# awikner/SPEEDY-ML-1

Measured on AMD Instinct MI355X. Metric: hybrid timesteps/sec, T30L8 + 1152x6k-node reservoirs; 1/2/4/8-GPU scaling, higher is better.
Workload: dtype f64

## Files before the change

### speedy-ml-1_amd/csrc/sml_dynamics.hip

```cpp
#include <hip/hip_runtime.h>

#include <array>
#include <cmath>
#include <cstddef>
#include <cstdlib>
#include <cstring>
#include <new>
#include <utility>
#include <vector>

#include "sml_dynamics_tables.hpp"
#include "sml_fft.hpp"
#include "sml_fft_wa96.hpp"
#include "sml_physics.hpp"
#include "sml_physics_pair.hpp"
#include "sml_spectral_internal.hpp"
#include "sml_timeline.hpp"

SML_TL_DEFINE(dynamics)

using namespace sml;

namespace {

// ... 385 lines not shown
    SML_TAB_NM(X)
#undef X
    __device__ double gradx_m() const { return t->gradx; }
    __device__ double xc(int k1, int k) const { return t->xc[k1][k]; }
    __device__ double xd(int k1, int k) const { return t->xd[k1][k]; }
    __device__ double xj(int n, int k1, int k) const { return t->xj[k1][k][n]; }
};

__host__ __device__ inline double tabm_value(const DynTables *__restrict__ T, int m, int i) {
    const TabM *z = nullptr;
    const size_t off = (size_t)i * sizeof(double);
#define X(name)                                                                             \
    {                                                                                       \
        const size_t a = offsetof(TabM, name), b = a + sizeof(z->name);                      \
        if (off >= a && off < b) return T->name[(off - a) / sizeof(double)];                 \
    }
    SML_TAB_VEC(X)
#undef X
#define X(name)                                                                             \
    {                                                                                       \
        const size_t a = offsetof(TabM, name), b = a + sizeof(z->name);                      \
        if (off >= a && off < b) return T->name[(off - a) / sizeof(double)][m];              \
    }
    SML_TAB_NM(X)
#undef X
    if (off >= offsetof(TabM, xc) && off < offsetof(TabM, xc) + sizeof(z->xc))
        return (&T->xc[0][0])[(off - offsetof(TabM, xc)) / sizeof(double)];
    if (off >= offsetof(TabM, xd) && off < offsetof(TabM, xd) + sizeof(z->xd))
        return (&T->xd[0][0])[(off - offsetof(TabM, xd)) / sizeof(double)];
    if (off == offsetof(TabM, gradx)) return T->gradx[m];
    if (off >= offsetof(TabM, xj)) {
        const int q = (int)((off - offsetof(TabM, xj)) / sizeof(double));
        const int k1 = q / (kKX * kNX), k = (q / kNX) % kKX, n = q % kNX;
        return m + n >= 1 ? T->xj[m + n - 1][k1][k] : 0.0;
    }
    return 0.0;
}

template <class U, class V, class TB>
__device__ inline void vds_gen(U u, V v, const TB &tb, int n, int p, double *vor, double *div) {
    const double gx = tb.gradx_m();
    const double ux = u(1 - p, n), vx = v(1 - p, n);
    const double zp = p == 1 ? gx * ux : -gx * ux;
    const double zc = p == 1 ? gx * vx : -gx * vx;
    static_assert(kNTRUN1 - 1 == kNX - 2, "vds's last row reads n - 1");
    const int nm = n > 0 ? n - 1 : 0, np = n < kNX - 1 ? n + 1 : kNX - 1;
    const double um = u(p, nm), up = u(p, np), vm = v(p, nm), vp = v(p, np);
    const double dym = tb.vddym_n(n), dyp = tb.vddyp_n(n);
    const double vor0 = zc - dyp * up, div0 = zp + dyp * vp;
    const double vorl = dym * um, divl = -dym * vm;
    const double vori = dym * um - dyp * up + zc, divi = -dym * vm + dyp * vp + zp;
    *vor = n == 0 ? vor0 : n == kNX - 1 ? vorl : vori;
    *div = n == 0 ? div0 : n == kNX - 1 ? divl : divi;
}

__device__ inline void vds_at(const double *u, const double *v, const DynTables *T, int m, int n, int p, double *vor,
                              double *div) {
    vds_gen([&](int pp, int nn) { return u[ci(pp, m, nn)]; }, [&](int pp, int nn) { return v[ci(pp, m, nn)]; },
            GTab{T, m}, n, p, vor, div);
}

__global__ void k_dyn_combine(const double *__restrict__ S, double *__restrict__ Td, const DynTables *__restrict__ T) {
    const int mn = blockIdx.x * blockDim.x + threadIdx.x;
    if (mn >= kMN) return;
    const int k = blockIdx.y;
    const int m = mn % kMX, n = mn / kMX;
    auto fld = [&](int f) { return S + (size_t)f * kSF; };
#pragma unroll
    for (int p = 0; p < 2; ++p) {
        const int c = ci(p, m, n);
        double vo, dv, d0, dq, dummy;
        vds_at(fld(k), fld(3 * kKX + k), T, m, n, p, &vo, &dv);
        const double lapv = -(fld(6 * kKX + k)[c] * T->el2[n][m]);
        Td[kTVor + (size_t)k * kSF + c] = vo;
        Td[kTDiv + (size_t)k * kSF + c] = dv - lapv;
        vds_at(fld(kKX + k), fld(4 * kKX + k), T, m, n, p, &dummy, &d0);
        Td[kTT + (size_t)k * kSF + c] = d0 + fld(7 * kKX + k)[c];
        vds_at(fld(2 * kKX + k), fld(5 * kKX + k), T, m, n, p, &dummy, &dq);
        Td[kTTr + (size_t)k * kSF + c] = dq + fld(8 * kKX + k)[c];
        if (k == 0) Td[kTPs + c] = (m == 0 && n == 0) ? 0.0 : fld(kNFwd - 1)[c];
    }
}

template <int CW, bool KU, class SA, class TB>
__device__ inline void tail_coef(SA S, double *__restrict__ Td, double *__restrict__ phi_out,
                                 const double *__restrict__ phis, const double *__restrict__ tcorh,
                                 const double *__restrict__ qcorh, int fc, const TB &tb,
                                 double (*sh)[kKX][CW], int cc, int k, int c, int m, int n, double vordt, double divdt,
                                 double tdt, double trdt, double psdt, int j1, int j4, double dt, double alph,
                                 double rob, double wil) {
    sh[0][k][cc] = S(1, j4, k);
    sh[1][k][cc] = S(2, j4, k);
    __syncthreads();
    double d0[kKX], dh[kKX], t1[kKX], g1[kKX], g2[kKX];
#pragma unroll
    for (int kk = 0; kk < kKX; ++kk) {
        d0[kk] = sh[0][kk][cc];
        dh[kk] = tb.dhs(kk);
        t1[kk] = sh[1][kk][cc];
        g1[kk] = tb.xgeop1(kk);
        g2[kk] = kk > 0 ? tb.xgeop2(kk) : 0.0;
    }
    const int km = k > 0 ? k - 1 : 0, kp = k < kKX - 1 ? k + 1 : kKX - 1;
    const double trk = tb.tref(k), trm = tb.tref(km), trp = tb.tref(kp), dhsr_k = tb.dhsr(k), tref3_k = tb.tref3(k),
                 tref2_k = tb.tref2(k), phis_c = phis[fc], corf_k = tb.corf(k);
    double dmeanc = 0.0;
#pragma unroll
    for (int kk = 0; kk < kKX; ++kk) dmeanc = dmeanc + d0[kk] * dh[kk];
    psdt = psdt - dmeanc;
    if (m == 0 && n == 0) psdt = 0.0;
    double sig_k = 0.0, sig_k1 = 0.0;
    if constexpr (KU) {
        double sg = 0.0, sgp = 0.0;
#pragma unroll
        for (int kk = 0; kk < kKX - 1; ++kk) {
            if (kk > k) break;
            const double nx_ = sg - dh[kk] * (d0[kk] - dmeanc);
            sgp = sg;
            sg = nx_;
        }
        if (k == kKX - 1) {
            sig_k = sg;
        } else {
            sig_k = sgp;
            sig_k1 = sg;
        }
    } else {
        double sg = 0.0;
#pragma unroll
        for (int kk = 0; kk < kKX - 1; ++kk) {
            const double nx_ = sg - dh[kk] * (d0[kk] - dmeanc);
            if (kk == k - 1) sig_k = nx_;
            if (kk == k) sig_k1 = nx_;
            sg = nx_;
        }
    }
    const double dumk_k = (k == 0) ? 0.0 : sig_k * (trk - trm);
    const double dumk_k1 = (k == kKX - 1) ? 0.0 : sig_k1 * (trp - trk);
    tdt = tdt - (dumk_k1 + dumk_k) * dhsr_k + tref3_k * (sig_k1 + sig_k) - tref2_k * dmeanc;
    double phi = phis_c + g1[kKX - 1] * t1[kKX - 1];
#pragma unroll
    for (int kk = kKX - 2; kk >= 0; --kk) {
        if constexpr (KU)
            if (kk < k) break;
        const double nx = phi + g2[kk + 1] * t1[kk + 1] + g1[kk] * t1[kk];
        phi = kk >= k ? nx : phi;
    }
    {
        const double pc = phi + corf_k * (sh[1][kp][cc] - sh[1][km][cc]);
        if (m == 0 && k >= 1 && k <= kKX - 2) phi = pc;
    }
    if (phi_out) phi_out[(size_t)k * kSF + c] = phi;
    {
        const double d1 = phi + kRgas * trk * S(4, j4, 0);
        const double lapd = -(d1 * tb.el2_n(n));
        divdt = divdt - lapd;
    }
    if (alph != 0.0) {
        sh[2][k][cc] = tdt;
        __syncthreads();
        double ye = 0.0;
#pragma unroll
        for (int k1 = 0; k1 < kKX; ++k1) ye = ye + tb.xd(k1, k) * sh[2][k1][cc];
        ye = ye + tb.tref1(k) * psdt;
        sh[1][k][cc] = divdt + tb.elz_n(n) * ye;
        __syncthreads();
        divdt = 0.0;
        const int ll = m + n;
        if (ll != 0) {
#pragma unroll
            for (int k1 = 0; k1 < kKX; ++k1) divdt = divdt + tb.xj(n, k1, k) * sh[1][k1][cc];
        }
        sh[0][k][cc] = divdt;
        __syncthreads();
#pragma unroll
        for (int kk = 0; kk < kKX; ++kk) psdt = psdt - sh[0][kk][cc] * tb.dhsx(kk);
#pragma unroll
        for (int k1 = 0; k1 < kKX; ++k1) tdt = tdt + tb.xc(k1, k) * sh[0][k1][cc];
    }
    const double dmp = tb.dmp_n(n), dmp1 = tb.dmp1_n(n), dmpd = tb.dmpd_n(n), dmp1d = tb.dmp1d_n(n);
    vordt = (vordt - dmp * S(0, 1, k)) * dmp1;
    divdt = (divdt - dmpd * S(1, 1, k)) * dmp1d;
    const double ctmp = S(2, 1, k) + tcorh[fc] * tb.tcorv(k);
    tdt = (tdt - dmp * ctmp) * dmp1;
    if (k == 0) {
        if (m == 0) {
            const double sdrag = 1. / (kTdrs * 3600.);
            vordt = vordt - sdrag * S(0, 1, 0);
            divdt = divdt - sdrag * S(1, 1, 0);
        }
        const double dmps = tb.dmps_n(n), dmp1s = tb.dmp1s_n(n);
        vordt = (vordt - dmps * S(0, 1, 0)) * dmp1s;
        divdt = (divdt - dmps * S(1, 1, 0)) * dmp1s;
        tdt = (tdt - dmps * ctmp) * dmp1s;
    }
    {
        const double cq = S(3, 1, k) + qcorh[fc] * tb.qcorv(k);
        trdt = (trdt - dmpd * cq) * dmp1d;
    }
    if (dt <= 0.0) {
        if (!Td) return;
        Td[kTVor + (size_t)k * kSF + c] = vordt;
        Td[kTDiv + (size_t)k * kSF + c] = divdt;
        Td[kTT + (size_t)k * kSF + c] = tdt;
        Td[kTTr + (size_t)k * kSF + c] = trdt;
        if (k == 0) Td[kTPs + c] = psdt;
        return;
    }
    const double eps = (j1 == 1) ? 0.0 : rob;
    const double trf = tb.trfilt_n(n);
    auto timint = [&](int var, int kk, double fdt) {
        fdt = fdt * trf;
        double &f1 = S(var, 1, kk);
        double &f2 = S(var, 2, kk);
        const double fj1_old = (j1 == 1) ? f1 : f2;
        const double fnew = f1 + dt * fdt;
        const double f1new = fj1_old + wil * eps * (f1 - 2 * fj1_old + fnew);
        const double fj1_new = (j1 == 1) ? f1new : fj1_old;
        f2 = fnew - (1 - wil) * eps * (f1new - 2 * fj1_new + fnew);
        f1 = f1new;
    };
    if (k == 0) timint(4, 0, psdt);
    timint(0, k, vordt);
    timint(1, k, divdt);
    timint(2, k, tdt);
    timint(3, k, trdt);
}

constexpr int kTailC = 32;
__global__ __launch_bounds__(256) void k_dyn_tail(double *__restrict__ st, double *__restrict__ Td,
                                                  double *__restrict__ phi_out, const double *__restrict__ phis,
                                                  const double *__restrict__ tcorh, const double *__restrict__ qcorh,
                                                  const DynTables *__restrict__ T, int j1, int j4, double dt,
                                                  double alph, double rob, double wil) {
    __shared__ double sh[3][kKX][kTailC];
    const int cc = threadIdx.x & (kTailC - 1), k = threadIdx.x / kTailC;
    const int c = blockIdx.x * kTailC + cc;
    const int mn = c >> 1, m = mn % kMX, n = mn / kMX;
    auto S = [&](int var, int lev, int kk) -> double & {
        if (var == 4) return st[kOffPs + (size_t)(lev - 1) * kSF + c];
        const size_t off = var == 0 ? kOffVor : var == 1 ? kOffDiv : var == 2 ? kOffT : kOffTr;
        return st[off + ((size_t)(lev - 1) * kKX + kk) * kSF + c];
    };
    tail_coef<kTailC, false>(S, Td, phi_out, phis, tcorh, qcorh, c, GTab{T, m}, sh, cc, k, c, m, n,
                             Td[kTVor + (size_t)k * kSF + c], Td[kTDiv + (size_t)k * kSF + c],
                             Td[kTT + (size_t)k * kSF + c], Td[kTTr + (size_t)k * kSF + c], Td[kTPs + c], j1, j4, dt,
                             alph, rob, wil);
}

typedef double d4 __attribute__((ext_vector_type(4)));
#define MFMA64(a, b, c) __builtin_amdgcn_mfma_f64_16x16x4f64((a), (b), (c), 0, 0, 0)

__device__ __attribute__((always_inline)) inline void store2(double *base, size_t idx, double a, double b) {
    *reinterpret_cast<double2 *>(base + idx) = double2{a, b};
}

constexpr int kCW = 2 * kNX;
static_assert(kCW == 64, "one level per 64-lane wave: wave_index() is the level index of the per-m kernels");
__device__ inline int wave_index() { return __builtin_amdgcn_readfirstlane((int)(threadIdx.x >> 6)); }
constexpr int kNIo = 4 * kKX + 1;
constexpr int kNIoWind = 2 * kKX;
constexpr int kSM = 5 * 2 * kKX * kCW;
constexpr int kVLs = 2 * kNFwd;
constexpr int kVFm = kIL * kVLs;
constexpr int kVIl = 2 * kNInvMax;
constexpr int kVIm = kIL * kVIl;
__device__ inline int smi(int var, int lev, int k, int cc) { return ((var * 2 + lev - 1) * kKX + k) * kCW + cc; }

constexpr int kStampKernels = 4, kStampBlocks = 96, kStamps = 8;
__device__ inline void stamp(long long *dbg, int kern, int i) {
    if (dbg && threadIdx.x == 0) dbg[((size_t)kern * kStampBlocks + blockIdx.x) * kStamps + i] = wall_clock64();
}

__global__ void k_state_to_m(const double *__restrict__ st, double *__restrict__ sm) {
    const int e = blockIdx.x * blockDim.x + threadIdx.x;
    if (e >= kMX * kSM) return;
    const int m = e / kSM, i = e % kSM;
    const int cc = i % kCW, k = (i / kCW) % kKX, lev = (i / (kCW * kKX)) % 2, var = i / (2 * kKX * kCW);
    const int c = ci(cc & 1, m, cc >> 1);
    double v = 0.0;
    if (var < 4) {
        const size_t off = var == 0 ? kOffVor : var == 1 ? kOffDiv : var == 2 ? kOffT : kOffTr;
        v = st[off + ((size_t)lev * kKX + k) * kSF + c];
    } else if (k == 0) {
        v = st[kOffPs + (size_t)lev * kSF + c];
    }
    sm[e] = v;
}

__device__ inline void put_state(double *__restrict__ st, int m, int i, double v) {
    const int cc = i % kCW, k = (i / kCW) % kKX, lev = (i / (kCW * kKX)) % 2, var = i / (2 * kKX * kCW);
    const int c = ci(cc & 1, m, cc >> 1);
    if (var < 4) {
        const size_t off = var == 0 ? kOffVor : var == 1 ? kOffDiv : var == 2 ? kOffT : kOffTr;
        st[off + ((size_t)lev * kKX + k) * kSF + c] = v;
    } else if (k == 0) {
        st[kOffPs + (size_t)lev * kSF + c] = v;
    }
}


template <class TB>
__device__ inline void uvspec_sel(const double *Sst, const TB &tb, int lev, int k, int n, int p, double *u,
                                  double *v) {
    static_assert(kNTRUN1 - 1 == kNX - 2, "uvspec's last row reads n - 1");
    const int nm = n > 0 ? n - 1 : 0, np = n < kNX - 1 ? n + 1 : kNX - 1;
    const bool first = n == 0, last = n == kNX - 1;
    const double vor_m = Sst[smi(0, lev, k, 2 * nm + p)], vor_p = Sst[smi(0, lev, k, 2 * np + p)];
    const double div_m = Sst[smi(1, lev, k, 2 * nm + p)], div_p = Sst[smi(1, lev, k, 2 * np + p)];
// ... 113 lines not shown
            accA = MFMA64(half ? gb.b11[s] : gb.b10[s], a1, accA);
        }
        if (!ok) continue;
        double *vr = varm + (size_t)m * kVIm + fa * 2 + p;
#pragma unroll
        for (int q = 0; q < 4; ++q) {
            const int j = 16 * half + kk + 4 * q;
            if (j >= kIY) continue;
            const double sym = accS[q], asym = accA[q];
            vr[(kIL - 1 - j) * kVIl] = sym + asym;
            vr[j * kVIl] = sym - asym;
        }
    }
}

__device__ inline void gridy_io(const double *In, const GridyB &gb, double *__restrict__ varm, int m, int nf) {
    const int wave = wave_index(), nw = blockDim.x >> 6;
    const int l = threadIdx.x & 63, r = l & 15, kk = l >> 4;
    for (int tile = wave; tile < (nf + 7) / 8; tile += nw) {
        const int f0 = tile * 8;
        const int fa = f0 + (r >> 1), p = r & 1;
        const bool ok = fa < nf;
        const double *a = In + (ok ? fa : 0) * kCW + p;
        d4 acc00 = {0, 0, 0, 0}, acc01 = acc00, acc10 = acc00, acc11 = acc00;
#pragma unroll
        for (int s = 0; s < 4; ++s) {
            const int n_odd = 2 * (4 * s + kk);
            const int n_even = n_odd + 1;
            const double a0 = ok ? a[2 * n_odd] : 0.0;
            const double a1 = ok ? a[2 * n_even] : 0.0;
            acc00 = MFMA64(a0, gb.b00[s], acc00);
            acc01 = MFMA64(a0, gb.b01[s], acc01);
            acc10 = MFMA64(a1, gb.b10[s], acc10);
            acc11 = MFMA64(a1, gb.b11[s], acc11);
        }
#pragma unroll
        for (int q = 0; q < 4; ++q) {
            const int row = kk + 4 * q;
            const int f = f0 + (row >> 1);
            if (f >= nf) continue;
            double *vr = varm + (size_t)f * kVarmField + 2 * m + (row & 1);
            {
                const int j = r;
                const double sym = acc00[q], asym = acc10[q];
                vr[(kIL - 1 - j) * kMX2] = sym + asym;
                vr[j * kMX2] = sym - asym;
            }
            const int j = 16 + r;
            if (j < kIY) {
                const double sym = acc01[q], asym = acc11[q];
                vr[(kIL - 1 - j) * kMX2] = sym + asym;
                vr[j * kMX2] = sym - asym;
            }
        }
    }
}

template <class TB, class Put>
__device__ inline void io_prep_m(const double *Sst, const TB &tb, int k, int cc, Put put) {
    const int n = cc >> 1, p = cc & 1;
    double a, b;
    uvspec_sel(Sst, tb, 1, k, n, p, &a, &b);
    put(k, a);
    put(kKX + k, b);
    put(2 * kKX + k, Sst[smi(2, 1, k, cc)]);
    put(3 * kKX + k, Sst[smi(3, 1, k, cc)]);
    if (k == 0) put(4 * kKX, Sst[smi(4, 1, 0, cc)]);
}

__device__ inline void load_forcing_m(double *Fm, const double *__restrict__ phis, const double *__restrict__ tcorh,
                                      const double *__restrict__ qcorh, int m) {
    for (int i = threadIdx.x; i < 3 * kCW; i += blockDim.x) {
        const int which = i / kCW, cc = i % kCW;
        const double *src = which == 0 ? phis : which == 1 ? tcorh : qcorh;
        Fm[i] = src[ci(cc & 1, m, cc >> 1)];
    }
}

constexpr int kSpecThreads = kCW * kKX;
constexpr int kSpecBlk = 512;
constexpr int kSpecSplit = 2;
#ifndef SML_SPEC_STRIDE
#define SML_SPEC_STRIDE 32
#endif
#ifndef SML_SPEC_VFM_FIRST
#define SML_SPEC_VFM_FIRST 0
#endif
constexpr int kSpecStride = SML_SPEC_STRIDE;
static_assert(kSpecStride >= kMX, "k_st_spec grid stride");

__global__ __launch_bounds__(kSpecThreads) void k_st_inv(const double *__restrict__ sm, const double *__restrict__ phis,
                                                         const DynTables *__restrict__ T,
                                                         const double *__restrict__ pinv, double *__restrict__ varm,
                                                         int j2, int n1, int nin) {
    __shared__ double Sst[kSM];
    __shared__ double In[kNInvMax * kCW];
    __shared__ double Fm[kCW];
    const int m = blockIdx.x;
    const double *src = sm + (size_t)m * kSM;
    for (int i = threadIdx.x; i < kSM / 2; i += blockDim.x)
        reinterpret_cast<double2 *>(Sst)[i] = reinterpret_cast<const double2 *>(src)[i];
    for (int cc = threadIdx.x; cc < kCW; cc += blockDim.x) Fm[cc] = phis[ci(cc & 1, m, cc >> 1)];
    __syncthreads();
    inv_inputs(Sst, In, Fm, GTab{T, m}, m, j2, n1, nin);
    __syncthreads();
    gridy_m(In, gridy_operands(pinv, m), varm, m, nin);
}

constexpr int kRowThreads = 128, kRowLd = 97;
static_assert(kNInvMax <= kRowThreads && kNFwd <= kRowThreads && kIX <= kRowThreads, "one thread per transform");

__device__ __attribute__((always_inline)) inline void row_gridx(double *A, const double *__restrict__ varm, const double *__restrict__ wa, int f,
                                 int j, bool kcos2, double cj) {
    const double *v = varm + (size_t)j * kVIl + f * 2;
    auto V = [&](int c) { return v[(size_t)(c >> 1) * kVIm + (c & 1)]; };
    double x[kFftN];
    x[0] = V(0);
#pragma unroll
    for (int e = 1; e <= kMX2 - 2; ++e) x[e] = V(e + 1);
#pragma unroll
    for (int e = kMX2 - 1; e < kFftN; ++e) x[e] = 0.0;
    fft::rfftb96_reg(x, wa);
#pragma unroll
    for (int e = 0; e < kFftN; ++e) A[e * kRowLd + f] = kcos2 ? x[e] * cj : x[e];
}

__device__ __attribute__((always_inline)) inline void row_specx(double *x, double *__restrict__ vfm, const double *__restrict__ wa, int f, int j) {
    fft::rfftf96_reg(x, wa);
    const double scale = 1. / (double)kIX;
    double *o = vfm + (size_t)j * kVLs + f * 2;
    o[0] = x[0] * scale;
    o[1] = 0.0;
#pragma unroll
    for (int c = 2; c < kMX2; ++c) o[(size_t)(c >> 1) * kVFm + (c & 1)] = x[c - 1] * scale;
}

__device__ __attribute__((always_inline)) inline void row_gridx_load(const double *__restrict__ varm, int f, int j,
                                                                     double (&xi)[kMX2 - 1]) {
    const double *v = varm + (size_t)j * kVIl + f * 2;
    xi[0] = v[0];
#pragma unroll
    for (int e = 1; e < kMX2 - 1; ++e) xi[e] = v[(size_t)((e + 1) >> 1) * kVIm + ((e + 1) & 1)];
    __builtin_amdgcn_sched_barrier(0);
}

__device__ __attribute__((always_inline)) inline void row_gridx_half(double *A, const double (&xi)[kMX2 - 1],
                                                                     const double *__restrict__ wa, int f,
                                                                     bool kcos2, double cj, int h) {
    double y[48];
    fft::rfftb96_half([&](int e) { return e <= kMX2 - 2 ? xi[e] : 0.0; }, h, y, wa);
#pragma unroll
    for (int q = 0; q < 48; ++q) A[(2 * q + h) * kRowLd + f] = kcos2 ? y[q] * cj : y[q];
}

__device__ __attribute__((always_inline)) inline void row_specx_pair(const double *x48, double *S, bool act,
                                                                     double *__restrict__ vfm,
                                                                     const double *__restrict__ wa, int f, int j,
                                                                     int h) {
    if (act) {
#pragma unroll
        for (int i = 0; i < 48; ++i) S[(48 * h + i) * kRowLd + f] = x48[i];
    }
    __syncthreads();
    if (!act) return;
    auto E = [&](int i) { return S[i * kRowLd + f]; };
    auto O = [&](int i) { return S[(48 + i) * kRowLd + f]; };
    const double scale = 1. / (double)kIX;
#pragma unroll
    for (int i = 0; i < 16; ++i) {
// ... 202 lines not shown
        SML_PST_T(18, 256);
        SML_PST_T(19, 384);
    }
    __syncthreads();
    SML_PST_T(20, 256);
    if (isp) {
        const double *Bh = B + pi * kRowLd + kNFwd;
        const double *Mh = mhs + pi * kMh;
        double *Bi = B + pi * kRowLd;
        const double rps = po.rps;
#pragma unroll
        for (int s = 0; s < 4; ++s) {
            const int k = 4 * ph_ + s;
            const double ttk = (k == 0 ? 0.0 : Bh[k > 0 ? k - 1 : 0]) + Mh[4 * ph_ + s] + po.rlw[s];
            double ttv = Bh[7 + k], utv = 0., vtv = 0.;
            double qtk;
            if (k == kKX - 1) {
                utv = utv + po.ust * rps * PTl->grdsig[kKX - 1];
                vtv = vtv + po.vst * rps * PTl->grdsig[kKX - 1];
                ttv = ttv + po.shf * rps * PTl->grdscp[kKX - 1];
                const double qtv = Bh[23] + po.evp * rps * PTl->grdsig[kKX - 1];
                qtk = Bh[22] + qtv;
            } else {
                qtk = Bh[15 + k];
            }
            Bi[k] = (Bi[k] + (0. + utv)) * cj;
            Bi[3 * kKX + k] = (Bi[3 * kKX + k] + (0. + vtv)) * cj;
            Bi[7 * kKX + k] = Bi[7 * kKX + k] + (ttk + ttv);
            Bi[8 * kKX + k] = Bi[8 * kKX + k] + qtk;
        }
    }
    __syncthreads();
    stamp(dbg, 0, 2);
    {
        const int f = tid >> 1, h = tid & 1;
        const bool act = f < kNFwd;
        double x[48];
        if (act) {
            const double *fr = B + f + h * kRowLd;
#pragma unroll
            for (int i = 0; i < 48; ++i) x[i] = fr[2 * i * kRowLd];
            fft::rfftf48_reg(x, was);
        }
        __syncthreads();
        row_specx_pair(x, A, act, vfm, was, f, j, h);
    }
    stamp(dbg, 0, 3);
}

__global__ void k_pack_pfwd(const double *__restrict__ pfwd, double *__restrict__ pfl) {
    const int e = blockIdx.x * blockDim.x + threadIdx.x;
    if (e >= kMX * (kIY / 4) * 64) return;
    const int l = e % 64, s = (e / 64) % (kIY / 4), m = e / (64 * (kIY / 4));
    const int r = l & 15, kk = l >> 4, j = 4 * s + kk;
    const double *pm = pfwd + (size_t)m * kNX * kIY;
    pfl[2 * (size_t)e] = pm[(2 * r) * kIY + j];
    pfl[2 * (size_t)e + 1] = pm[(2 * r + 1) * kIY + j];
}

__global__ __launch_bounds__(kSpecBlk) void k_st_spec(
    const double *__restrict__ vfm, const double *__restrict__ pfl, const double *__restrict__ wt,
    const double *__restrict__ sm, double *__restrict__ sm_out, double *__restrict__ Td, double *__restrict__ phi_out,
    const double *__restrict__ phis,
    const double *__restrict__ tcorh, const double *__restrict__ qcorh, const DynTables *__restrict__ T, int j1,
    int j4, double dt, double alph, double rob, double wil, const double *__restrict__ pinv,
    double *__restrict__ varm_next, int next_j2, int n1, int nin, const double *__restrict__ tabm,
    double *__restrict__ state_out, double *__restrict__ io_varm, long long *dbg) {
    SML_TL_SCOPE(sml::tl::kSpec);
    __shared__ double V[kVFm];
    __shared__ double S[kNInvMax * kCW];
    __shared__ double sh[3][kKX][kCW];
    __shared__ double Sst[kSM];
    __shared__ double Fm[3 * kCW];
    const int m = blockIdx.x % kSpecStride, half = blockIdx.x / kSpecStride;
    if (m >= kMX) return;
    const bool lead = half == 0;
    if (!lead) dbg = nullptr;
    const int wave = wave_index(), l = threadIdx.x & 63, r = l & 15, kk = l >> 4;
    const int sk = next_j2 > 0 ? 1 : 3;
    stamp(dbg, sk, 0);
    const double *vm = vfm + (size_t)m * kVFm;
    constexpr int kTiles = (kNFwd + 7) / 8, kWaves = kSpecBlk / 64;
    static_assert(kTiles <= 2 * kWaves, "specy: two tiles per wave at most");
    auto tile_load = [&](int tile, double (&vn)[kIY / 4], double (&vs)[kIY / 4]) {
        const int fa = tile * 8 + (r >> 1);
        const double *vr = vm + (fa < kNFwd ? fa : 0) * 2 + (r & 1);
#pragma unroll
        for (int s = 0; s < kIY / 4; ++s) {
            const int j = 4 * s + kk;
            vn[s] = vr[(kIL - 1 - j) * kVLs];
            vs[s] = vr[j * kVLs];
        }
    };
    double vn0[kIY / 4], vs0[kIY / 4], vn1[kIY / 4], vs1[kIY / 4];
    const bool two = wave + kWaves < kTiles;
#if SML_SPEC_VFM_FIRST
    tile_load(wave, vn0, vs0);
    if (two) tile_load(wave + kWaves, vn1, vs1);
#endif
    constexpr int RT = (kTabMDoubles / 2 + kSpecBlk - 1) / kSpecBlk;
    static_assert((RT == 2 || RT == 3) && 2 * RT * kSpecBlk <= kVFm && 2 * RT * kSpecBlk - kTabMDoubles <= kTabMPad,
                  "TabM staging");
    double2 rt0, rt1, rt2 = {0.0, 0.0};
    constexpr int NS = kSM / 2, RS = (NS + kSpecBlk - 1) / kSpecBlk;
    static_assert(RS == 5 && NS % kSpecBlk == 0, "state staging: five whole rows of the block");
    double2 rs0, rs1, rs2, rs3, rs4;
    {
        const double2 *ss = reinterpret_cast<const double2 *>(sm + (size_t)m * kSM) + threadIdx.x;
        rs0 = ss[0];
        rs1 = ss[kSpecBlk];
        rs2 = ss[2 * kSpecBlk];
        rs3 = ss[3 * kSpecBlk];
        rs4 = ss[4 * kSpecBlk];
        const double2 *t = reinterpret_cast<const double2 *>(tabm + (size_t)m * kTabMDoubles) + threadIdx.x;
        rt0 = t[0];
        rt1 = t[kSpecBlk];
        if constexpr (RT > 2) rt2 = t[2 * kSpecBlk];
    }
    double rf = 0.0;
    if (threadIdx.x < 3 * kCW) {
        const int which = threadIdx.x / kCW, cf = threadIdx.x % kCW;
        const double *src = which == 0 ? phis : which == 1 ? tcorh : qcorh;
        rf = src[ci(cf & 1, m, cf >> 1)];
    }
    constexpr int kPinvM = kNX * 32, kVPinv = 2 * RT * kSpecBlk;
    static_assert(kPinvM == 2 * kSpecBlk && kVPinv + kPinvM <= kVFm && kVPinv % 2 == 0, "pinv slice staging in V");
    const double2 rp = reinterpret_cast<const double2 *>(pinv + (size_t)m * kPinvM)[threadIdx.x];
    const double2 *pl = reinterpret_cast<const double2 *>(pfl) + (size_t)m * (kIY / 4) * 64 + l;
    double wv[kIY / 4], bS[kIY / 4], bD[kIY / 4];
#pragma unroll
    for (int s = 0; s < kIY / 4; ++s) {
        const double2 b = pl[s * 64];
        wv[s] = wt[4 * s + kk];
        bS[s] = b.x;
        bD[s] = b.y;
    }
    if (dbg) __syncthreads();
    stamp(dbg, sk, 1);
    auto tile_mma = [&](int tile, const double (&vn)[kIY / 4], const double (&vs)[kIY / 4]) {
        const int f0 = tile * 8;
        d4 accS = {0, 0, 0, 0}, accD = accS;
#pragma unroll
        for (int s = 0; s < kIY / 4; ++s) {
            const double aS = (vn[s] + vs[s]) * wv[s];
            const double aD = (vn[s] - vs[s]) * wv[s];
            accS = MFMA64(aS, bS[s], accS);
            accD = MFMA64(aD, bD[s], accD);
        }
#pragma unroll
        for (int q = 0; q < 4; ++q) {
            const int row = kk + 4 * q;
            const int f = f0 + (row >> 1);
            if (f >= kNFwd) continue;
            S[f * kCW + 2 * (2 * r) + (row & 1)] = accS[q];
            S[f * kCW + 2 * (2 * r + 1) + (row & 1)] = accD[q];
        }
    };
    {
#if !SML_SPEC_VFM_FIRST
        tile_load(wave, vn0, vs0);
        if (two) tile_load(wave + kWaves, vn1, vs1);
#endif
        tile_mma(wave, vn0, vs0);
        if (two) tile_mma(wave + kWaves, vn1, vs1);
    }
    TabM *tm = reinterpret_cast<TabM *>(V);
    {
        double2 *v2 = reinterpret_cast<double2 *>(V) + threadIdx.x;
        v2[0] = rt0;
        v2[kSpecBlk] = rt1;
        if constexpr (RT > 2) v2[2 * kSpecBlk] = rt2;
        double2 *s2 = reinterpret_cast<double2 *>(Sst) + threadIdx.x;
        s2[0] = rs0;
        s2[kSpecBlk] = rs1;
        s2[2 * kSpecBlk] = rs2;
        s2[3 * kSpecBlk] = rs3;
        s2[4 * kSpecBlk] = rs4;
        if (threadIdx.x < 3 * kCW) Fm[threadIdx.x] = rf;
        reinterpret_cast<double2 *>(V + kVPinv)[threadIdx.x] = rp;
    }
    __syncthreads();
    const LTab tb{tm};
    stamp(dbg, sk, 2);
    static_assert(kSpecBlk == kSpecThreads, "k_st_spec: one thread per (coefficient, level), none idle in the tail");
    const int cc = threadIdx.x & (kCW - 1), k = wave;
    const int n = cc >> 1, p = cc & 1;
    const int c = ci(p, m, n);
    auto fl = [&](int f) { return [=](int pp, int nn) { return S[f * kCW + 2 * nn + pp]; }; };
    double vo = 0.0, dv = 0.0, d0 = 0.0, dq = 0.0, dummy;
    vds_gen(fl(k), fl(3 * kKX + k), tb, n, p, &vo, &dv);
    const double lapv = -(fl(6 * kKX + k)(p, n) * tb.el2_n(n));
    vds_gen(fl(kKX + k), fl(4 * kKX + k), tb, n, p, &dummy, &d0);
    vds_gen(fl(2 * kKX + k), fl(5 * kKX + k), tb, n, p, &dummy, &dq);
    const double psdt = (m == 0 && n == 0) ? 0.0 : fl(kNFwd - 1)(p, n);
    const double tdt0 = d0 + fl(7 * kKX + k)(p, n), trdt0 = dq + fl(8 * kKX + k)(p, n);
    if (dbg) {
        __syncthreads();
        stamp(dbg, sk, 3);
    }
    auto SA = [&](int var, int lev, int kk2) -> double & { return Sst[smi(var, lev, kk2, cc)]; };
    tail_coef<kCW, true>(SA, lead ? Td : nullptr, lead && next_j2 <= 0 ? phi_out : nullptr, Fm, Fm + kCW, Fm + 2 * kCW,
                         cc, tb, sh, cc, k, c, m, n, vo, dv - lapv, tdt0, trdt0, psdt, j1, j4, dt, alph, rob, wil);
    __syncthreads();
    stamp(dbg, sk, 4);
    if (next_j2 <= 0) {
        if (!lead) return;
        for (int i = threadIdx.x; i < kSM; i += kSpecBlk) put_state(state_out, m, i, Sst[i]);
        if (io_varm) {
            io_prep_m(Sst, tb, k, cc, [&](int f, double v) { S[f * kCW + cc] = v; });
            __syncthreads();
            gridy_io(S, gridy_operands_slice(V + kVPinv), io_varm, m, kNIo);
        }
        return;
    }
    if (lead) {
        const double2 *src = reinterpret_cast<const double2 *>(Sst) + threadIdx.x;
        double2 v[RS];
#pragma unroll
        for (int q = 0; q < RS; ++q) v[q] = src[q * kSpecBlk];
#pragma unroll
        for (int q = 0; q < RS; ++q)
            store2(sm_out, (size_t)m * kSM + 2 * ((size_t)q * kSpecBlk + threadIdx.x), v[q].x, v[q].y);
    }
    inv_inputs(Sst, S, Fm, tb, m, next_j2, n1, nin);
    __syncthreads();
    stamp(dbg, sk, 5);
    {
        const int nt = (nin + 7) / 8, per = (nt + kSpecSplit - 1) / kSpecSplit;
        gridy_m(S, gridy_operands_slice(V + kVPinv), varm_next, m, nin, half * per, min(nt, (half + 1) * per));
    }
    if (dbg) {
        __syncthreads();
        stamp(dbg, sk, 6);
    }
}



__global__ void k_io_combine(const double *__restrict__ S, double *__restrict__ st, const DynTables *__restrict__ T) {
    const int mn = blockIdx.x * blockDim.x + threadIdx.x;
    if (mn >= kMN) return;
    const int k = blockIdx.y;
    const int m = mn % kMX, n = mn / kMX;
    const double trf = T->trfilt[n][m];
#pragma unroll
    for (int p = 0; p < 2; ++p) {
        const int c = ci(p, m, n);
        double vo, dv;
        vds_at(S + (size_t)k * kSF, S + (size_t)(kKX + k) * kSF, T, m, n, p, &vo, &dv);
        st[kOffVor + (size_t)k * kSF + c] = vo * trf;
        st[kOffDiv + (size_t)k * kSF + c] = dv * trf;
        st[kOffT + (size_t)k * kSF + c] = S[(size_t)(2 * kKX + k) * kSF + c] * trf;
        st[kOffTr + (size_t)k * kSF + c] = S[(size_t)(3 * kKX + k) * kSF + c] * trf;
        if (k == 0) st[kOffPs + c] = S[(size_t)(4 * kKX) * kSF + c] * trf;
    }
}

__global__ void k_io_prep(const double *__restrict__ st, double *__restrict__ sin_, const DynTables *__restrict__ T) {
    const int mn = blockIdx.x * blockDim.x + threadIdx.x;
    if (mn >= kMN) return;
    const int k = blockIdx.y;
    const int m = mn % kMX, n = mn / kMX;
    const double *vor = st + kOffVor + (size_t)k * kSF, *div = st + kOffDiv + (size_t)k * kSF;
    uvspec_at(vor, div, T, m, n, sin_ + (size_t)k * kSF, sin_ + (size_t)(kKX + k) * kSF);
#pragma unroll
    for (int p = 0; p < 2; ++p) {
        const int c = ci(p, m, n);
        sin_[(size_t)(2 * kKX + k) * kSF + c] = st[kOffT + (size_t)k * kSF + c];
        sin_[(size_t)(3 * kKX + k) * kSF + c] = st[kOffTr + (size_t)k * kSF + c];
        if (k == 0) sin_[(size_t)(4 * kKX) * kSF + c] = st[kOffPs + c];
    }
}

__global__ __launch_bounds__(kSpecThreads) void k_io_entry(const double *__restrict__ vio,
                                                           const double *__restrict__ pfl,
                                                           const double *__restrict__ wt, double *__restrict__ state,
                                                           double *__restrict__ sm, double *__restrict__ chk,
                                                           const double *__restrict__ phis,
                                                           const double *__restrict__ tabm,
                                                           const double *__restrict__ pinv, double *__restrict__ varm,
                                                           int n1, int nin, uint64_t *__restrict__ xa, uint64_t xa0,
                                                           uint64_t xa1) {
    SML_TL_SCOPE(sml::tl::kIoEntry);
    if (xa && blockIdx.x == 0 && threadIdx.x == 0) {
        xa[0] = xa0;
// ... 1381 lines not shown
```

Measured before the change: 1212.

## Split tail into pre/post and overlap vfm tile loads with state-only tail work

Splits the spectral tail into a state-only prologue (sigma, geopotential, damping corrections) and a post part that needs the Legendre results. In the fused spectral kernel the prologue now runs before the MFMA Legendre step, interleaved with global tile loads: half the waves load first and the rest load after the prologue, to hide load latency. Legendre columns and weights are staged in shared memory instead of per-thread global loads, and the pinv slice store moves after the MFMA step. Adds sched barriers and an extra register-held TailPre struct, which may raise register pressure.

```diff
diff --git a/speedy-ml-1_amd/csrc/sml_dynamics.hip b/speedy-ml-1_amd/csrc/sml_dynamics.hip
--- a/speedy-ml-1_amd/csrc/sml_dynamics.hip
+++ b/speedy-ml-1_amd/csrc/sml_dynamics.hip
@@ -491,33 +491,29 @@
     }
 }
 
-template <int CW, bool KU, class SA, class TB>
-__device__ inline void tail_coef(SA S, double *__restrict__ Td, double *__restrict__ phi_out,
-                                 const double *__restrict__ phis, const double *__restrict__ tcorh,
-                                 const double *__restrict__ qcorh, int fc, const TB &tb,
-                                 double (*sh)[kKX][CW], int cc, int k, int c, int m, int n, double vordt, double divdt,
-                                 double tdt, double trdt, double psdt, int j1, int j4, double dt, double alph,
-                                 double rob, double wil) {
-    sh[0][k][cc] = S(1, j4, k);
-    sh[1][k][cc] = S(2, j4, k);
-    __syncthreads();
+struct TailPre {
+    double dmeanc, sig_k, sig_k1, dumk_k, dumk_k1, lapd, ctmp, cq;
+};
+
+template <bool KU, class SA, class LV, class TB>
+__device__ inline TailPre tail_pre(SA S, LV L, double *__restrict__ phi_out, const double *__restrict__ phis,
+                                   const double *__restrict__ tcorh, const double *__restrict__ qcorh, int fc,
+                                   const TB &tb, int k, int c, int m, int n, int j4) {
+    TailPre r;
     double d0[kKX], dh[kKX], t1[kKX], g1[kKX], g2[kKX];
 #pragma unroll
     for (int kk = 0; kk < kKX; ++kk) {
-        d0[kk] = sh[0][kk][cc];
+        d0[kk] = L(0, kk);
         dh[kk] = tb.dhs(kk);
-        t1[kk] = sh[1][kk][cc];
+        t1[kk] = L(1, kk);
         g1[kk] = tb.xgeop1(kk);
         g2[kk] = kk > 0 ? tb.xgeop2(kk) : 0.0;
     }
     const int km = k > 0 ? k - 1 : 0, kp = k < kKX - 1 ? k + 1 : kKX - 1;
-    const double trk = tb.tref(k), trm = tb.tref(km), trp = tb.tref(kp), dhsr_k = tb.dhsr(k), tref3_k = tb.tref3(k),
-                 tref2_k = tb.tref2(k), phis_c = phis[fc], corf_k = tb.corf(k);
+    const double trk = tb.tref(k), trm = tb.tref(km), trp = tb.tref(kp), phis_c = phis[fc], corf_k = tb.corf(k);
     double dmeanc = 0.0;
 #pragma unroll
     for (int kk = 0; kk < kKX; ++kk) dmeanc = dmeanc + d0[kk] * dh[kk];
-    psdt = psdt - dmeanc;
-    if (m == 0 && n == 0) psdt = 0.0;
     double sig_k = 0.0, sig_k1 = 0.0;
     if constexpr (KU) {
         double sg = 0.0, sgp = 0.0;
@@ -544,9 +540,11 @@
             sg = nx_;
         }
     }
-    const double dumk_k = (k == 0) ? 0.0 : sig_k * (trk - trm);
-    const double dumk_k1 = (k == kKX - 1) ? 0.0 : sig_k1 * (trp - trk);
-    tdt = tdt - (dumk_k1 + dumk_k) * dhsr_k + tref3_k * (sig_k1 + sig_k) - tref2_k * dmeanc;
+    r.dmeanc = dmeanc;
+    r.sig_k = sig_k;
+    r.sig_k1 = sig_k1;
+    r.dumk_k = (k == 0) ? 0.0 : sig_k * (trk - trm);
+    r.dumk_k1 = (k == kKX - 1) ? 0.0 : sig_k1 * (trp - trk);
     double phi = phis_c + g1[kKX - 1] * t1[kKX - 1];
 #pragma unroll
     for (int kk = kKX - 2; kk >= 0; --kk) {
@@ -556,15 +554,31 @@
         phi = kk >= k ? nx : phi;
     }
     {
-        const double pc = phi + corf_k * (sh[1][kp][cc] - sh[1][km][cc]);
+        const double pc = phi + corf_k * (L(1, kp) - L(1, km));
         if (m == 0 && k >= 1 && k <= kKX - 2) phi = pc;
     }
     if (phi_out) phi_out[(size_t)k * kSF + c] = phi;
     {
         const double d1 = phi + kRgas * trk * S(4, j4, 0);
-        const double lapd = -(d1 * tb.el2_n(n));
-        divdt = divdt - lapd;
-    }
+        r.lapd = -(d1 * tb.el2_n(n));
+    }
+    r.ctmp = S(2, 1, k) + tcorh[fc] * tb.tcorv(k);
+    r.cq = S(3, 1, k) + qcorh[fc] * tb.qcorv(k);
+    return r;
+}
+
+template <int CW, class SA, class TB>
+__device__ inline void tail_post(SA S, const TailPre &pre, double *__restrict__ Td, const TB &tb,
+                                 double (*sh)[kKX][CW], int cc, int k, int c, int m, int n, double vordt, double divdt,
+                                 double tdt, double trdt, double psdt, int j1, double dt, double alph, double rob,
+                                 double wil) {
+    const double dmeanc = pre.dmeanc, sig_k = pre.sig_k, sig_k1 = pre.sig_k1, dumk_k = pre.dumk_k,
+                 dumk_k1 = pre.dumk_k1, ctmp = pre.ctmp;
+    const double dhsr_k = tb.dhsr(k), tref3_k = tb.tref3(k), tref2_k = tb.tref2(k);
+    psdt = psdt - dmeanc;
+    if (m == 0 && n == 0) psdt = 0.0;
+    tdt = tdt - (dumk_k1 + dumk_k) * dhsr_k + tref3_k * (sig_k1 + sig_k) - tref2_k * dmeanc;
+    divdt = divdt - pre.lapd;
     if (alph != 0.0) {
         sh[2][k][cc] = tdt;
         __syncthreads();
@@ -590,7 +604,6 @@
     const double dmp = tb.dmp_n(n), dmp1 = tb.dmp1_n(n), dmpd = tb.dmpd_n(n), dmp1d = tb.dmp1d_n(n);
     vordt = (vordt - dmp * S(0, 1, k)) * dmp1;
     divdt = (divdt - dmpd * S(1, 1, k)) * dmp1d;
-    const double ctmp = S(2, 1, k) + tcorh[fc] * tb.tcorv(k);
     tdt = (tdt - dmp * ctmp) * dmp1;
     if (k == 0) {
         if (m == 0) {
@@ -603,10 +616,7 @@
         divdt = (divdt - dmps * S(1, 1, 0)) * dmp1s;
         tdt = (tdt - dmps * ctmp) * dmp1s;
     }
-    {
-        const double cq = S(3, 1, k) + qcorh[fc] * tb.qcorv(k);
-        trdt = (trdt - dmpd * cq) * dmp1d;
-    }
+    trdt = (trdt - dmpd * pre.cq) * dmp1d;
     if (dt <= 0.0) {
         if (!Td) return;
         Td[kTVor + (size_t)k * kSF + c] = vordt;
@@ -634,6 +644,21 @@
     timint(1, k, divdt);
     timint(2, k, tdt);
     timint(3, k, trdt);
+}
+
+template <int CW, bool KU, class SA, class TB>
+__device__ inline void tail_coef(SA S, double *__restrict__ Td, double *__restrict__ phi_out,
+                                 const double *__restrict__ phis, const double *__restrict__ tcorh,
+                                 const double *__restrict__ qcorh, int fc, const TB &tb,
+                                 double (*sh)[kKX][CW], int cc, int k, int c, int m, int n, double vordt, double divdt,
+                                 double tdt, double trdt, double psdt, int j1, int j4, double dt, double alph,
+                                 double rob, double wil) {
+    sh[0][k][cc] = S(1, j4, k);
+    sh[1][k][cc] = S(2, j4, k);
+    __syncthreads();
+    const TailPre pre = tail_pre<KU>(S, [&](int v, int kk) { return sh[v][kk][cc]; }, phi_out, phis, tcorh, qcorh, fc,
+                                     tb, k, c, m, n, j4);
+    tail_post<CW>(S, pre, Td, tb, sh, cc, k, c, m, n, vordt, divdt, tdt, trdt, psdt, j1, dt, alph, rob, wil);
 }
 
 constexpr int kTailC = 32;
@@ -913,9 +938,6 @@
 constexpr int kSpecSplit = 2;
 #ifndef SML_SPEC_STRIDE
 #define SML_SPEC_STRIDE 32
-#endif
-#ifndef SML_SPEC_VFM_FIRST
-#define SML_SPEC_VFM_FIRST 0
 #endif
 constexpr int kSpecStride = SML_SPEC_STRIDE;
 static_assert(kSpecStride >= kMX, "k_st_spec grid stride");
@@ -1284,6 +1306,7 @@
     const double *vm = vfm + (size_t)m * kVFm;
     constexpr int kTiles = (kNFwd + 7) / 8, kWaves = kSpecBlk / 64;
     static_assert(kTiles <= 2 * kWaves, "specy: two tiles per wave at most");
+    static_assert(kTiles - kWaves <= kWaves / 2, "specy: the waves with two tiles are among those that load first");
     auto tile_load = [&](int tile, double (&vn)[kIY / 4], double (&vs)[kIY / 4]) {
         const int fa = tile * 8 + (r >> 1);
         const double *vr = vm + (fa < kNFwd ? fa : 0) * 2 + (r & 1);
@@ -1296,10 +1319,6 @@
     };
     double vn0[kIY / 4], vs0[kIY / 4], vn1[kIY / 4], vs1[kIY / 4];
     const bool two = wave + kWaves < kTiles;
-#if SML_SPEC_VFM_FIRST
-    tile_load(wave, vn0, vs0);
-    if (two) tile_load(wave + kWaves, vn1, vs1);
-#endif
     constexpr int RT = (kTabMDoubles / 2 + kSpecBlk - 1) / kSpecBlk;
     static_assert((RT == 2 || RT == 3) && 2 * RT * kSpecBlk <= kVFm && 2 * RT * kSpecBlk - kTabMDoubles <= kTabMPad,
                   "TabM staging");
@@ -1326,46 +1345,19 @@
         rf = src[ci(cf & 1, m, cf >> 1)];
     }
     constexpr int kPinvM = kNX * 32, kVPinv = 2 * RT * kSpecBlk;
-    static_assert(kPinvM == 2 * kSpecBlk && kVPinv + kPinvM <= kVFm && kVPinv % 2 == 0, "pinv slice staging in V");
+    constexpr int kPflM = 2 * (kIY / 4) * 64, kVPfl = kVPinv + kPinvM, kVWt = kVPfl + kPflM;
+    static_assert(kPinvM == 2 * kSpecBlk && kVPinv % 2 == 0, "pinv slice staging in V");
+    static_assert(kPflM / 2 <= kSpecBlk && kIY <= 64 && kVWt + kIY <= kVFm, "Legendre columns and weights staged in V");
+    double2 rl = {0.0, 0.0};
+    double rw = 0.0;
+    if (threadIdx.x < kPflM / 2)
+        rl = reinterpret_cast<const double2 *>(pfl)[(size_t)m * (kPflM / 2) + threadIdx.x];
+    if (threadIdx.x < kIY) rw = wt[threadIdx.x];
+    __builtin_amdgcn_sched_barrier(0);
     const double2 rp = reinterpret_cast<const double2 *>(pinv + (size_t)m * kPinvM)[threadIdx.x];
-    const double2 *pl = reinterpret_cast<const double2 *>(pfl) + (size_t)m * (kIY / 4) * 64 + l;
-    double wv[kIY / 4], bS[kIY / 4], bD[kIY / 4];
-#pragma unroll
-    for (int s = 0; s < kIY / 4; ++s) {
-        const double2 b = pl[s * 64];
-        wv[s] = wt[4 * s + kk];
-        bS[s] = b.x;
-        bD[s] = b.y;
-    }
+    __builtin_amdgcn_sched_barrier(0);
     if (dbg) __syncthreads();
     stamp(dbg, sk, 1);
-    auto tile_mma = [&](int tile, const double (&vn)[kIY / 4], const double (&vs)[kIY / 4]) {
-        const int f0 = tile * 8;
-        d4 accS = {0, 0, 0, 0}, accD = accS;
-#pragma unroll
-        for (int s = 0; s < kIY / 4; ++s) {
-            const double aS = (vn[s] + vs[s]) * wv[s];
-            const double aD = (vn[s] - vs[s]) * wv[s];
-            accS = MFMA64(aS, bS[s], accS);
-            accD = MFMA64(aD, bD[s], accD);
-        }
-#pragma unroll
-        for (int q = 0; q < 4; ++q) {
-            const int row = kk + 4 * q;
-            const int f = f0 + (row >> 1);
-            if (f >= kNFwd) continue;
-            S[f * kCW + 2 * (2 * r) + (row & 1)] = accS[q];
-            S[f * kCW + 2 * (2 * r + 1) + (row & 1)] = accD[q];
-        }
-    };
-    {
-#if !SML_SPEC_VFM_FIRST
-        tile_load(wave, vn0, vs0);
-        if (two) tile_load(wave + kWaves, vn1, vs1);
-#endif
-        tile_mma(wave, vn0, vs0);
-        if (two) tile_mma(wave + kWaves, vn1, vs1);
-    }
     TabM *tm = reinterpret_cast<TabM *>(V);
     {
         double2 *v2 = reinterpret_cast<double2 *>(V) + threadIdx.x;
@@ -1379,15 +1371,60 @@
         s2[3 * kSpecBlk] = rs3;
         s2[4 * kSpecBlk] = rs4;
         if (threadIdx.x < 3 * kCW) Fm[threadIdx.x] = rf;
-        reinterpret_cast<double2 *>(V + kVPinv)[threadIdx.x] = rp;
+        if (threadIdx.x < kPflM / 2) reinterpret_cast<double2 *>(V + kVPfl)[threadIdx.x] = rl;
+        if (threadIdx.x < kIY) V[kVWt + threadIdx.x] = rw;
     }
     __syncthreads();
     const LTab tb{tm};
-    stamp(dbg, sk, 2);
     static_assert(kSpecBlk == kSpecThreads, "k_st_spec: one thread per (coefficient, level), none idle in the tail");
     const int cc = threadIdx.x & (kCW - 1), k = wave;
     const int n = cc >> 1, p = cc & 1;
     const int c = ci(p, m, n);
+    auto SA = [&](int var, int lev, int kk2) -> double & { return Sst[smi(var, lev, kk2, cc)]; };
+    const bool loads_first = wave < kWaves / 2;
+    if (loads_first) {
+        tile_load(wave, vn0, vs0);
+        if (two) tile_load(wave + kWaves, vn1, vs1);
+    }
+    __builtin_amdgcn_sched_barrier(0);
+    const TailPre pre = tail_pre<true>(SA, [&](int v, int kk2) { return Sst[smi(1 + v, j4, kk2, cc)]; },
+                                       lead && next_j2 <= 0 ? phi_out : nullptr, Fm, Fm + kCW, Fm + 2 * kCW, cc, tb, k,
+                                       c, m, n, j4);
+    __builtin_amdgcn_sched_barrier(0);
+    if (!loads_first) tile_load(wave, vn0, vs0);
+    __builtin_amdgcn_sched_barrier(0);
+    double wv[kIY / 4], bS[kIY / 4], bD[kIY / 4];
+#pragma unroll
+    for (int s = 0; s < kIY / 4; ++s) {
+        const double2 b = reinterpret_cast<const double2 *>(V + kVPfl)[s * 64 + l];
+        wv[s] = V[kVWt + 4 * s + kk];
+        bS[s] = b.x;
+        bD[s] = b.y;
+    }
+    auto tile_mma = [&](int tile, const double (&vn)[kIY / 4], const double (&vs)[kIY / 4]) {
+        const int f0 = tile * 8;
+        d4 accS = {0, 0, 0, 0}, accD = accS;
+#pragma unroll
+        for (int s = 0; s < kIY / 4; ++s) {
+            const double aS = (vn[s] + vs[s]) * wv[s];
+            const double aD = (vn[s] - vs[s]) * wv[s];
+            accS = MFMA64(aS, bS[s], accS);
+            accD = MFMA64(aD, bD[s], accD);
+        }
+#pragma unroll
+        for (int q = 0; q < 4; ++q) {
+            const int row = kk + 4 * q;
+            const int f = f0 + (row >> 1);
+            if (f >= kNFwd) continue;
+            S[f * kCW + 2 * (2 * r) + (row & 1)] = accS[q];
+            S[f * kCW + 2 * (2 * r + 1) + (row & 1)] = accD[q];
+        }
+    };
+    tile_mma(wave, vn0, vs0);
+    if (two) tile_mma(wave + kWaves, vn1, vs1);
+    reinterpret_cast<double2 *>(V + kVPinv)[threadIdx.x] = rp;
+    __syncthreads();
+    stamp(dbg, sk, 2);
     auto fl = [&](int f) { return [=](int pp, int nn) { return S[f * kCW + 2 * nn + pp]; }; };
     double vo = 0.0, dv = 0.0, d0 = 0.0, dq = 0.0, dummy;
     vds_gen(fl(k), fl(3 * kKX + k), tb, n, p, &vo, &dv);
@@ -1400,9 +1437,8 @@
         __syncthreads();
         stamp(dbg, sk, 3);
     }
-    auto SA = [&](int var, int lev, int kk2) -> double & { return Sst[smi(var, lev, kk2, cc)]; };
-    tail_coef<kCW, true>(SA, lead ? Td : nullptr, lead && next_j2 <= 0 ? phi_out : nullptr, Fm, Fm + kCW, Fm + 2 * kCW,
-                         cc, tb, sh, cc, k, c, m, n, vo, dv - lapv, tdt0, trdt0, psdt, j1, j4, dt, alph, rob, wil);
+    tail_post<kCW>(SA, pre, lead ? Td : nullptr, tb, sh, cc, k, c, m, n, vo, dv - lapv, tdt0, trdt0, psdt, j1, dt, alph,
+                   rob, wil);
     __syncthreads();
     stamp(dbg, sk, 4);
     if (next_j2 <= 0) {
```

New measurement: 1232, median of 6. 1.02x the previous value.
